# wondmgezahu/RAMP

Measured on AMD Instinct MI355X. Metric: sampled trajectories/sec (H=48, T=25), higher is better.
Workload: dtype f32-emulated (2 x fp16 planes per operand, fp32 accumulate)

## Files before the change

ramp_amd/csrc/tkc.hip:

```cpp
#include "args_conv.h"
#include "tokmma.h"

#include <algorithm>

namespace ramp {

namespace {

constexpr int tc_xrows(int NG) { return NG == 4 ? 64 + 2 + 2 : 48 + 2 * 6 + 2; }
constexpr int tc_scr(int NG) { return NG == 4 ? 2304 : 2048; }

__device__ __forceinline__ float tc_mish(float x) {
  const float e = __builtin_amdgcn_exp2f(fminf(x, 20.f) * 1.44269504088896340736f);
  const float n = e * (e + 2.f);
  return x * (n * __builtin_amdgcn_rcpf(n + 2.f));
}
__device__ __forceinline__ float tc_mish_grad(float x) {
  const float e = __builtin_amdgcn_exp2f(fminf(x, 20.f) * 1.44269504088896340736f);
  const float n = e * (e + 2.f);
  const float w = __builtin_amdgcn_rcpf(n + 2.f);
  return n * w + x * (4.f * e * (e + 1.f) * w * w);
}

__device__ __forceinline__ f32x4 tc_mm32(const u32x4 a, const u32x4 b, const f32x4 c) {
  return __builtin_amdgcn_mfma_f32_16x16x32_f16(__builtin_bit_cast(half8, a), __builtin_bit_cast(half8, b), c, 0, 0, 0);
}
__device__ __forceinline__ void tc_wave_sync() {
  __builtin_amdgcn_fence(__ATOMIC_ACQ_REL, "wavefront");
  __builtin_amdgcn_wave_barrier();
}

}

__global__ void tkc_pack_kernel(const float* __restrict__ W, unsigned short* __restrict__ out, int N, int K, float scale) {
  const int total = 5 * (N / 16) * (K / 32) * 64;
  const int idx = blockIdx.x * 256 + threadIdx.x;
  if (idx >= total) return;
  const int lane = idx & 63, f = idx >> 6;
  const int j = f % (K / 32), nb = (f / (K / 32)) % (N / 16), tap = f / ((K / 32) * (N / 16));
  const float* src = W + ((long)tap * N + 16 * nb + (lane & 15)) * K + 32 * j + 8 * (lane >> 4);
  unsigned short* o = out + (long)f * 1024 + lane * 8;
#pragma unroll
  for (int e = 0; e < 8; ++e) {
    const float x = src[e] * scale;
    const _Float16 hi = (_Float16)x, lo = (_Float16)(x - (float)hi);
    o[e] = __builtin_bit_cast(unsigned short, hi); o[512 + e] = __builtin_bit_cast(unsigned short, lo);
  }
}
int tkc_pack(const float* W, int N, int K, float scale, unsigned short* out, hipStream_t s) {
  RAMP_REQUIRE(W && out && N % 16 == 0 && K % 32 == 0 && N >= 16 && N <= 64 && K >= 32 && K <= 64, "tkc_pack: bad shape");
  const int total = 5 * (N / 16) * (K / 32) * 64;
  hipLaunchKernelGGL(tkc_pack_kernel, dim3((total + 255) / 256), dim3(256), 0, s, W, out, N, K, scale);
  RAMP_HIP_CHECK(hipGetLastError());
  return 0;
}
size_t tkc_packed_halves(int N, int K) { return (size_t)5 * (N / 16) * (K / 32) * 1024; }

template <int NG, int NB, int KS, int PRO, int EPI>
__global__ __launch_bounds__(256) __attribute__((amdgpu_waves_per_eu(1, 2)))
void tkc_kernel(TkcArgs a, int n_tiles) {
  constexpr int T = 16 * NG, K = 32 * KS, N = 16 * NB;
  constexpr int XROW = 4 * K + 16;
  constexpr int WBYTES = 5 * NB * KS * 2048;
  constexpr int TC_XROWS = tc_xrows(NG), TC_SCR = tc_scr(NG);
  static_assert(8 * T * 4 + 8 * (NG == 4 ? 1 : 6) * 4 <= TC_SCR, "GroupNorm scratch");
  extern __shared__ __attribute__((aligned(16))) char smem[];
  const int tid = threadIdx.x, lane = tid & 63;
  const int wave = __builtin_amdgcn_readfirstlane(tid >> 6);
  const int c = lane & 15, g = lane >> 4;
  const int n_my = (n_tiles - (int)blockIdx.x + (int)gridDim.x - 1) / (int)gridDim.x;

  const bool exact = a.amax_in == nullptr;
  float s_in = scale_of(a.amax_in);
  float os = a.wsi / s_in;
  float amax = 0.f;

  for (int i = tid; i < WBYTES / 16; i += 256) reinterpret_cast<u32x4*>(smem)[i] = reinterpret_cast<const u32x4*>(a.W)[i];
  char* xt = smem + WBYTES + wave * (TC_XROWS * XROW);
  for (int i = lane; i < TC_XROWS * XROW / 16; i += 64) reinterpret_cast<u32x4*>(xt)[i] = u32x4{0u, 0u, 0u, 0u};
  float* const wscr = reinterpret_cast<float*>(smem + WBYTES + 4 * (TC_XROWS * XROW) + wave * TC_SCR);
  __syncthreads();

  int xrow[NG], smp[NG];
#pragma unroll
  for (int t = 0; t < NG; ++t) { smp[t] = (16 * t + c) / a.L; xrow[t] = (16 * t + c) + 2 * smp[t] + 2; }
  const int n_smp = T / a.L;
  auto tok_sums = [&](float (&v)[4][NG], int nblk, int C) __attribute__((always_inline)) {
    const int gsz = C >> 3;
#pragma unroll
    for (int b = 0; b < 4; ++b) {
      if (b < nblk) {
#pragma unroll
        for (int t = 0; t < NG; ++t) {
          float q = v[b][t];
          if (gsz == 8) q += __shfl_xor(q, 16);
          const int grp = gsz == 4 ? 4 * b + g : 2 * b + (g >> 1);
          if (gsz == 4 || !(g & 1)) wscr[grp * T + 16 * t + c] = q;
        }
      }
    }
    tc_wave_sync();
    if (lane < 8 * n_smp) {
      const int grp = lane / n_smp, sm = lane - grp * n_smp;
      double q = 0.0;
      for (int u = 0; u < a.L; ++u) q += (double)wscr[grp * T + sm * a.L + u];
      wscr[8 * T + lane] = (float)(q / (double)(a.L * gsz));
    }
    tc_wave_sync();
#pragma unroll
    for (int b = 0; b < 4; ++b) {
      if (b < nblk) {
#pragma unroll
        for (int t = 0; t < NG; ++t) {
          const int grp = gsz == 4 ? 4 * b + g : 2 * b + (g >> 1);
          v[b][t] = wscr[8 * T + grp * n_smp + smp[t]];
        }
      }
    }
    tc_wave_sync();
  };
  const int m_last = a.M - 1;
  const char* xbase = reinterpret_cast<const char*>(a.X);

  f32x4 xr[K / 16][NG];
  f32x4 cr[PRO ? K / 16 : 1][PRO ? NG : 1];
  float gmu[PRO ? K / 16 : 1][PRO ? NG : 1], grs[PRO ? K / 16 : 1][PRO ? NG : 1];
  auto load_x = [&](int tile) __attribute__((always_inline)) {
    int tk0 = tile * (4 * T) + wave * T + c;
    asm volatile("" : "+v"(tk0));
#pragma unroll
    for (int t = 0; t < NG; ++t) {
      const unsigned tk = (unsigned)min(tk0 + 16 * t, m_last);
      const char* row = xbase + ((size_t)tk * (unsigned)(4 * a.ldx) + 16u * (unsigned)g);
#pragma unroll
      for (int fb = 0; fb < K / 16; ++fb) xr[fb][t] = *reinterpret_cast<const f32x4*>(row + 64 * fb);
      if constexpr (PRO) {
        const char* crow = reinterpret_cast<const char*>(a.gn_c) + ((size_t)tk * (unsigned)(4 * K) + 16u * (unsigned)g);
        const unsigned srow = tk / (unsigned)a.L;
#pragma unroll
        for (int fb = 0; fb < K / 16; ++fb) {
          cr[fb][t] = *reinterpret_cast<const f32x4*>(crow + 64 * fb);
          const int grp = K == 32 ? 4 * fb + g : 2 * fb + (g >> 1);
          gmu[fb][t] = a.gn_stats[((size_t)srow * 8 + grp) * 2]; grs[fb][t] = a.gn_stats[((size_t)srow * 8 + grp) * 2 + 1];
        }
      }
// ... 136 lines not shown
          var[nb][t] = q;
        }
      tok_sums(var, NB, N);
#pragma unroll
      for (int nb = 0; nb < NB; ++nb) {
        const f32x4 gam = *reinterpret_cast<const f32x4*>(a.gamma + 16 * nb + 4 * g), bet = *reinterpret_cast<const f32x4*>(a.beta + 16 * nb + 4 * g);
        f32x4 tb = (EPI == 1 && a.tbias) ? *reinterpret_cast<const f32x4*>(a.tbias + 16 * nb + 4 * g) : f32x4{0.f, 0.f, 0.f, 0.f};
#pragma unroll
        for (int t = 0; t < NG; ++t) {
          if constexpr (EPI == 2) tb = *reinterpret_cast<const f32x4*>(tline[t] + 16 * nb);
          const float rstd = 1.f / sqrtf(var[nb][t] + a.eps);
          const bool live = full || tok0 + 16 * t + c < a.M;
          if (live && (16 * t + c) - smp[t] * a.L == 0 && (N == 32 || !(g & 1))) {
            const int grp = N == 32 ? 4 * nb + g : 2 * nb + (g >> 1);
            float* st = a.stats + ((size_t)(trow[t] / (unsigned)a.L) * 8 + grp) * 2;
            st[0] = mean[nb][t]; st[1] = rstd;
          }
          f32x4 v;
#pragma unroll
          for (int j = 0; j < 4; ++j) v[j] = tc_mish((acc[nb][t][j] - mean[nb][t]) * rstd * gam[j] + bet[j]) + tb[j];
          if (a.resid) v += *reinterpret_cast<const f32x4*>(a.resid + (size_t)trow[t] * a.ldr + 16 * nb + 4 * g);
          if (live) *reinterpret_cast<f32x4*>(a.Y + (size_t)trow[t] * a.ldy + 16 * nb + 4 * g) = v;
        }
      }
    } else {
    {
      unsigned trow[NG];
#pragma unroll
      for (int t = 0; t < NG; ++t) trow[t] = (unsigned)min(tok0 + 16 * t + c, m_last);
      f32x4 bq[NB];
#pragma unroll
      for (int nb = 0; nb < NB; ++nb) bq[nb] = a.bias ? *reinterpret_cast<const f32x4*>(a.bias + 16 * nb + 4 * g) : f32x4{0.f, 0.f, 0.f, 0.f};
      if (full) {
        f32x4 rz[NB][NG];
#pragma unroll
        for (int nb = 0; nb < NB; ++nb)
#pragma unroll
          for (int t = 0; t < NG; ++t) rz[nb][t] = f32x4{0.f, 0.f, 0.f, 0.f};
        if (a.resid) {
#pragma unroll
          for (int nb = 0; nb < NB; ++nb)
#pragma unroll
            for (int t = 0; t < NG; ++t) rz[nb][t] = *reinterpret_cast<const f32x4*>(a.resid + (size_t)trow[t] * a.ldr + 16 * nb + 4 * g);
        }
        if (a.resid2) {
#pragma unroll
          for (int nb = 0; nb < NB; ++nb)
#pragma unroll
            for (int t = 0; t < NG; ++t) rz[nb][t] += *reinterpret_cast<const f32x4*>(a.resid2 + (size_t)trow[t] * a.ldr2 + 16 * nb + 4 * g);
        }
#pragma unroll
        for (int nb = 0; nb < NB; ++nb)
#pragma unroll
          for (int t = 0; t < NG; ++t) *reinterpret_cast<f32x4*>(a.Y + (size_t)trow[t] * a.ldy + 16 * nb + 4 * g) = acc[nb][t] * os + bq[nb] + rz[nb][t];
      } else {
#pragma unroll
        for (int nb = 0; nb < NB; ++nb)
#pragma unroll
          for (int t = 0; t < NG; ++t) {
            f32x4 v = acc[nb][t] * os + bq[nb];
            if (a.resid) v += *reinterpret_cast<const f32x4*>(a.resid + (size_t)trow[t] * a.ldr + 16 * nb + 4 * g);
            if (a.resid2) v += *reinterpret_cast<const f32x4*>(a.resid2 + (size_t)trow[t] * a.ldr2 + 16 * nb + 4 * g);
            if (tok0 + 16 * t + c < a.M) *reinterpret_cast<f32x4*>(a.Y + (size_t)trow[t] * a.ldy + 16 * nb + 4 * g) = v;
          }
      }
    }
  }

    }
  amax = fmaxf(amax, __shfl_xor(amax, 32)); amax = fmaxf(amax, __shfl_xor(amax, 16)); amax = fmaxf(amax, __shfl_xor(amax, 8));
  amax = fmaxf(amax, __shfl_xor(amax, 4)); amax = fmaxf(amax, __shfl_xor(amax, 2)); amax = fmaxf(amax, __shfl_xor(amax, 1));
  __syncthreads();
  record_amax_block_guarded<true>(a.amax_out, amax, reinterpret_cast<float*>(smem + WBYTES), exact ? nullptr : a.range_flag, s_in, a.site);
}

bool tkc_applicable(int M, int L, int N, int K, int* ng) {
  int n = 0;
  if (L >= 8 && 48 % L == 0) n = 3; else if (L >= 8 && 32 % L == 0) n = 2; else if (L == 64 && !(N == 64 && K == 64)) n = 4;
  if (ng) *ng = n;
  return n != 0 && M > 0 && M % L == 0 && (N == 32 || N == 64) && (K == 32 || K == 64);
}

namespace {
template <int NG, int NB, int KS> size_t tkc_lds() { return (size_t)5 * NB * KS * 2048 + 4 * (size_t)tc_xrows(NG) * (4 * 32 * KS + 16) + 4 * tc_scr(NG); }
template <int NG, int NB, int KS, int PRO, int EPI> int tkc_go(const TkcArgs& a, int n_tiles, hipStream_t s) {
  const size_t lds = tkc_lds<NG, NB, KS>();
  const int per_cu = lds * 2 <= 160 * 1024 ? 2 : 1;
  const int nb = std::min(n_tiles, per_cu * device_cu_count());
  hipLaunchKernelGGL((tkc_kernel<NG, NB, KS, PRO, EPI>), dim3(nb), dim3(256), lds, s, a, n_tiles);
  RAMP_HIP_CHECK(hipGetLastError());
  return 0;
}
}

int launch_tkc(const TkcArgs& a, hipStream_t s) {
  auto al16 = [](const void* p) { return (reinterpret_cast<uintptr_t>(p) & 15) == 0; };
  int ng = 0;
  RAMP_REQUIRE(tkc_applicable(a.M, a.L, a.N, a.K, &ng), "tkc: C_in, C_out in {32, 64}, tokens per sample >= 8 dividing 48 or 32 (or 64, not 64 x 64 channels), whole samples");
  RAMP_REQUIRE(a.X && a.W && a.Y && (a.dir == 1 || a.dir == -1), "tkc: bad operand");
  RAMP_REQUIRE(al16(a.X) && al16(a.W) && al16(a.Y) && al16(a.bias) && al16(a.resid) && al16(a.resid2) && a.ldx % 4 == 0 && a.ldy % 4 == 0 &&
               a.ldr % 4 == 0 && a.ldr2 % 4 == 0 && a.ldx >= a.K && a.ldy >= a.N, "tkc: operands must be 16-byte aligned");
  RAMP_REQUIRE((long)a.M * a.ldx * 4 < (1l << 32), "tkc: 32-bit row offsets");
  RAMP_REQUIRE(!ranges_overlap(a.Y, ((size_t)(a.M - 1) * a.ldy + a.N) * 4, a.X, ((size_t)(a.M - 1) * a.ldx + a.K) * 4), "tkc: the output must not overlap the operand");
  const int T = 16 * ng, n_tiles = (a.M + 4 * T - 1) / (4 * T);
  const int pro = a.gn_c ? 1 : 0, epi = a.Cst ? (a.t_rows ? 2 : 1) : 0;
  RAMP_REQUIRE(!a.t_rows || (a.Cst && a.tbias && a.tt_stride > 0 && a.tt_stride % 4 == 0), "tkc: a row -> timestep table needs the GroupNorm epilogue, the time table and its stride (a multiple of 4 floats)");
  RAMP_REQUIRE(!(pro && epi), "tkc: the GroupNorm backward operand and the GroupNorm epilogue do not occur together");
  if (pro) RAMP_REQUIRE(a.gn_stats && a.gn_gamma && a.gn_beta && al16(a.gn_c) && al16(a.gn_gamma) && al16(a.gn_beta) && a.ldx >= a.K, "tkc: GroupNorm-backward operand incomplete");
  if (epi) RAMP_REQUIRE(a.stats && a.gamma && a.beta && a.bias && !a.resid2 && al16(a.Cst) && al16(a.gamma) && al16(a.beta) && al16(a.tbias), "tkc: GroupNorm epilogue incomplete");
#define TC_SHAPE(NGV, PROV, EPIV) \
    if (a.N == 64 && a.K == 64) return tkc_go<NGV, 4, 2, PROV, EPIV>(a, n_tiles, s); \
    if (a.N == 64 && a.K == 32) return tkc_go<NGV, 4, 1, PROV, EPIV>(a, n_tiles, s); \
    if (a.N == 32 && a.K == 64) return tkc_go<NGV, 2, 2, PROV, EPIV>(a, n_tiles, s); \
    return tkc_go<NGV, 2, 1, PROV, EPIV>(a, n_tiles, s);
#define TC_CASE(NGV) \
  if (ng == NGV) { \
    if (pro) { TC_SHAPE(NGV, 1, 0) } \
    if (epi == 2) { TC_SHAPE(NGV, 0, 2) } \
    if (epi) { TC_SHAPE(NGV, 0, 1) } \
    TC_SHAPE(NGV, 0, 0) \
  }
  TC_CASE(3) TC_CASE(2)
#undef TC_SHAPE
#define TC_SHAPE(NGV, PROV, EPIV) \
    if (a.N == 64 && a.K == 32) return tkc_go<NGV, 4, 1, PROV, EPIV>(a, n_tiles, s); \
    if (a.N == 32 && a.K == 64) return tkc_go<NGV, 2, 2, PROV, EPIV>(a, n_tiles, s); \
    if (a.N == 32 && a.K == 32) return tkc_go<NGV, 2, 1, PROV, EPIV>(a, n_tiles, s);
  TC_CASE(4)
#undef TC_CASE
#undef TC_SHAPE
  RAMP_REQUIRE(false, "tkc: variant not built");
}

int init_tkc_attributes() {
#define TC_ATTR1(NGV, NBV, KSV, PROV, EPIV) RAMP_HIP_CHECK(hipFuncSetAttribute(reinterpret_cast<const void*>(&tkc_kernel<NGV, NBV, KSV, PROV, EPIV>), hipFuncAttributeMaxDynamicSharedMemorySize, (int)tkc_lds<NGV, NBV, KSV>()))
#define TC_ATTR(NGV, NBV, KSV) TC_ATTR1(NGV, NBV, KSV, 0, 0); TC_ATTR1(NGV, NBV, KSV, 1, 0); TC_ATTR1(NGV, NBV, KSV, 0, 1); TC_ATTR1(NGV, NBV, KSV, 0, 2)
  TC_ATTR(3, 4, 2); TC_ATTR(3, 4, 1); TC_ATTR(3, 2, 2); TC_ATTR(3, 2, 1);
  TC_ATTR(2, 4, 2); TC_ATTR(2, 4, 1); TC_ATTR(2, 2, 2); TC_ATTR(2, 2, 1);
  TC_ATTR(4, 4, 1); TC_ATTR(4, 2, 2); TC_ATTR(4, 2, 1);
#undef TC_ATTR
#undef TC_ATTR1
  return 0;
}

}
```

ramp_amd/csrc/tkw.hip:

```cpp
#include "args_conv.h"
#include "tokmma.h"

#include <algorithm>

namespace ramp {

namespace {

constexpr int TW_TB = 96;
constexpr int TW_NT = 3;
constexpr int TW_SCRATCH = 4096 + 4 * 1024;

__device__ __forceinline__ float tw_mish(float x) {
  const float e = __builtin_amdgcn_exp2f(fminf(x, 20.f) * 1.44269504088896340736f);
  const float n = e * (e + 2.f);
  return x * (n * __builtin_amdgcn_rcpf(n + 2.f));
}
__device__ __forceinline__ float tw_mish_grad(float x) {
  const float e = __builtin_amdgcn_exp2f(fminf(x, 20.f) * 1.44269504088896340736f);
  const float n = e * (e + 2.f);
  const float w = __builtin_amdgcn_rcpf(n + 2.f);
  return n * w + x * (4.f * e * (e + 1.f) * w * w);
}
__device__ __forceinline__ void tw_wave_sync() {
  __builtin_amdgcn_fence(__ATOMIC_ACQ_REL, "wavefront");
  __builtin_amdgcn_wave_barrier();
}

struct TwGeom { int KC, n_chunks, rows, xrow, n_pass; size_t lds; };
#define LR_GROUPS_OK(KC_, K_) (((KC_) / 4) / ((K_) / 32) <= 8)

}

template <int MB, int PRO, int EPI, bool RT>
__device__ __forceinline__ void tkw_body(const TkwArgs& a, int n_tiles, int kc32, int n_chunks, int n_rows, int n_pass, int mulL) {
  extern __shared__ __attribute__((aligned(16))) char smem[];
  const int tid = threadIdx.x, lane = tid & 63;
  const int wave = __builtin_amdgcn_readfirstlane(tid >> 6);
  const int tok = lane & 31, kh = lane >> 5;
  const int KC = kc32 << 5;
  const int XROW = 4 * KC + 16;
  const int KS = KC >> 4;
  char* const scr = smem + (size_t)n_rows * XROW;
  float* const wscr = reinterpret_cast<float*>(scr + wave * 1024);

  const float s_in = scale_of(a.amax_in);
  const float os = a.wsi / s_in;
  float amax = 0.f;
  auto divL = [&](int t) __attribute__((always_inline)) { return (t * mulL) >> 16; };
  auto trow = [&](int t) __attribute__((always_inline)) { return t + 2 * divL(t) + 2; };

  for (int i = tid; i < n_rows * XROW / 16; i += 256) reinterpret_cast<u32x4*>(smem)[i] = u32x4{0u, 0u, 0u, 0u};
  float* const prm = reinterpret_cast<float*>(scr + 4096);
  auto load_prm = [&](int c0) __attribute__((always_inline)) {
    for (int i = tid; i < min(a.N, 256); i += 256) {
      const int c = c0 + i;
      prm[i] = a.bias[c]; prm[256 + i] = a.gamma[c]; prm[512 + i] = a.beta[c]; prm[768 + i] = a.tbias ? a.tbias[c] : 0.f;
    }
  };
  if (EPI >= 1) load_prm(0);
  __syncthreads();

  int boff[TW_NT];
#pragma unroll
  for (int tg = 0; tg < TW_NT; ++tg) boff[tg] = trow(32 * tg + tok) * XROW + 16 * kh;
  const int LR = KC >> 2;
  const int RP = 64 / LR;
  const int sl = lane % LR, sr = lane / LR;
  const int m_last = a.M - 1;

#pragma unroll 1
  for (int tile = (int)blockIdx.x; tile < n_tiles; tile += (int)gridDim.x) {
    const int tok0 = tile * TW_TB;
#pragma unroll 1
    for (int pass = 0; pass < n_pass; ++pass) {
      f32x16 acc[MB][TW_NT];
#pragma unroll
      for (int mb = 0; mb < MB; ++mb)
#pragma unroll
        for (int tg = 0; tg < TW_NT; ++tg)
#pragma unroll
          for (int i = 0; i < 16; ++i) acc[mb][tg][i] = 0.f;
      const int nb0 = pass * 128 * MB + wave * 32 * MB;

#pragma unroll 1
      for (int kc = 0; kc < n_chunks; ++kc) {
        if (pass > 0 || kc > 0 || tile != (int)blockIdx.x) __syncthreads();
        if (EPI == 2 && kc == 0 && (pass > 0 || tile != (int)blockIdx.x)) load_prm(pass * 256);
        if (n_chunks > 1 || pass == 0) {
          const int ch = kc * KC + 4 * sl;
          if constexpr (PRO == 0) {
#pragma unroll 1
            for (int it0 = 0; it0 < 24; it0 += 8 * RP) {
              f32x4 v[8];
#pragma unroll
              for (int u = 0; u < 8; ++u) {
                const int t = 24 * wave + it0 + u * RP + sr;
                const int tk = min(tok0 + t, m_last);
                const float* src = ch < a.K1 ? a.X + (size_t)tk * a.ldx + ch : a.X2 + (size_t)tk * a.ldx2 + (ch - a.K1);
                v[u] = (it0 + u * RP < 24 && !(a.ablate & 2)) ? *reinterpret_cast<const f32x4*>(src) : f32x4{0.f, 0.f, 0.f, 0.f};
              }
#pragma unroll
              for (int u = 0; u < 8; ++u) {
                if (it0 + u * RP < 24) {
                  const int t = 24 * wave + it0 + u * RP + sr;
                  const f32x4 x = (tok0 + t < a.M) ? v[u] : f32x4{0.f, 0.f, 0.f, 0.f};
                  amax = amax4(x, amax);
                  unsigned h0, h1, l0, l1;
                  split4(x * s_in, h0, h1, l0, l1);
                  char* dst = smem + trow(t) * XROW + 8 * sl;
                  *reinterpret_cast<u32x2*>(dst) = u32x2{h0, h1};
                  *reinterpret_cast<u32x2*>(dst + 2 * KC) = u32x2{l0, l1};
                }
              }
            }
          } else {
            constexpr int NW = PRO > 0 ? PRO : 1;
            const int G4 = (a.K >> 5);
            const int grp = ch / (a.K >> 3), gl = sl / G4;
            const int n_gl = LR / G4;
            const f32x4 gam = *reinterpret_cast<const f32x4*>(a.gn_gamma + ch), bet = *reinterpret_cast<const f32x4*>(a.gn_beta + ch);
            const float inv_cnt = 1.f / (float)(a.L * (a.K >> 3));
            const int n_it = a.L / RP;
            const int spp = NW / n_it;
            const int n_smp = TW_TB / a.L;
            const int sm_lo = (wave * n_smp) >> 2, sm_hi = ((wave + 1) * n_smp) >> 2;
#pragma unroll 1
            for (int sm0 = sm_lo; sm0 < sm_hi; sm0 += spp) {
              const int t_lo = sm0 * a.L;
              f32x4 dv[NW], hv[NW];
              float mu[NW], rs[NW];
              int u_s = 0, u_i = 0;
#pragma unroll
              for (int u = 0; u < NW; ++u) {
                const int tk = min(tok0 + t_lo + u * RP + sr, m_last);
                dv[u] = *reinterpret_cast<const f32x4*>(a.X + (size_t)tk * a.ldx + ch);
                hv[u] = *reinterpret_cast<const f32x4*>(a.gn_c + (size_t)tk * a.K + ch);
                const int srow = min(tok0 / a.L + sm0 + u_s, m_last / a.L);
                mu[u] = a.gn_stats[((size_t)srow * 8 + grp) * 2]; rs[u] = a.gn_stats[((size_t)srow * 8 + grp) * 2 + 1];
                if (++u_i == n_it) { u_i = 0; ++u_s; }
              }
              float p1[NW], p2[NW];
#pragma unroll
              for (int u = 0; u < NW; ++u) {
                float s1 = 0.f, s2 = 0.f;
#pragma unroll
                for (int j = 0; j < 4; ++j) {
                  const float h = (hv[u][j] - mu[u]) * rs[u];
                  const float d = dv[u][j] * tw_mish_grad(h * gam[j] + bet[j]) * gam[j];
                  hv[u][j] = h; dv[u][j] = d;
                  s1 += d; s2 += d * h;
                }
                p1[u] = s1; p2[u] = s2;
              }
              for (int b = 1; b < G4; b <<= 1) {
#pragma unroll
                for (int u = 0; u < NW; ++u) { p1[u] += __shfl_xor(p1[u], b); p2[u] += __shfl_xor(p2[u], b); }
              }
              for (int b = LR; b < 64; b <<= 1) {
#pragma unroll
                for (int u = 0; u < NW; ++u) { p1[u] += __shfl_xor(p1[u], b); p2[u] += __shfl_xor(p2[u], b); }
              }
              if (sr == 0 && sl == gl * G4) {
#pragma unroll
                for (int u = 0; u < NW; ++u) { wscr[(gl * 8 + u) * 2] = p1[u]; wscr[(gl * 8 + u) * 2 + 1] = p2[u]; }
              }
              tw_wave_sync();
              if (lane < n_gl * spp) {
                const int g2 = lane / spp, s2i = lane - g2 * spp;
                float t1 = 0.f, t2 = 0.f;
                for (int i2 = 0; i2 < n_it; ++i2) { t1 += wscr[(g2 * 8 + s2i * n_it + i2) * 2]; t2 += wscr[(g2 * 8 + s2i * n_it + i2) * 2 + 1]; }
                wscr[(g2 * 8 + s2i * n_it) * 2] = t1 * inv_cnt; wscr[(g2 * 8 + s2i * n_it) * 2 + 1] = t2 * inv_cnt;
              }
              tw_wave_sync();
              u_s = 0; u_i = 0;
#pragma unroll
              for (int u = 0; u < NW; ++u) {
                const float m1 = wscr[(gl * 8 + u_s * n_it) * 2], m2 = wscr[(gl * 8 + u_s * n_it) * 2 + 1];
                if (++u_i == n_it) { u_i = 0; ++u_s; }
                const int t = t_lo + u * RP + sr;
                const bool live = tok0 + t < a.M;
                f32x4 x;
#pragma unroll
                for (int j = 0; j < 4; ++j) x[j] = live ? (dv[u][j] - m1 - hv[u][j] * m2) * rs[u] : 0.f;
                amax = amax4(x, amax);
                unsigned h0, h1, l0, l1;
                split4(x * s_in, h0, h1, l0, l1);
                char* dst = smem + trow(t) * XROW + 8 * sl;
                *reinterpret_cast<u32x2*>(dst) = u32x2{h0, h1};
                *reinterpret_cast<u32x2*>(dst + 2 * KC) = u32x2{l0, l1};
              }
              tw_wave_sync();
            }
          }
        }
        __syncthreads();

        const int n_steps = 5 * KS;
        const int lks = 31 - __builtin_clz(KS);
        const size_t wtap = (size_t)(a.N >> 5) * (a.K >> 4) * 2048;
        const char* wbase = reinterpret_cast<const char*>(a.W) + ((size_t)(nb0 >> 5) * (a.K >> 4) + (size_t)kc * KS) * 2048 + lane * 16;
        const size_t wmb = (size_t)(a.K >> 4) * 2048;
        auto load_a = [&](u32x4 (&h)[MB], u32x4 (&l)[MB], int st) __attribute__((always_inline)) {
          const char* p = wbase + (size_t)(st >> lks) * wtap + (size_t)(st & (KS - 1)) * 2048;
#pragma unroll
          for (int mb = 0; mb < MB; ++mb) {
            h[mb] = *reinterpret_cast<const u32x4*>(p + mb * wmb);
            l[mb] = *reinterpret_cast<const u32x4*>(p + mb * wmb + 1024);
          }
        };
        auto load_b = [&](u32x4 (&h)[TW_NT], u32x4 (&l)[TW_NT], int st) __attribute__((always_inline)) {
          const int sh = a.dir * ((st >> lks) - 2) * XROW + 32 * (st & (KS - 1));
#pragma unroll
          for (int tg = 0; tg < TW_NT; ++tg) {
            const char* p = smem + boff[tg] + sh;
            h[tg] = *reinterpret_cast<const u32x4*>(p);
            l[tg] = *reinterpret_cast<const u32x4*>(p + 2 * KC);
          }
        };
        auto step = [&](const u32x4 (&uah)[MB], const u32x4 (&ual)[MB], const u32x4 (&ubh)[TW_NT], const u32x4 (&ubl)[TW_NT],
                        u32x4 (&nah)[MB], u32x4 (&nal)[MB], u32x4 (&nbh)[TW_NT], u32x4 (&nbl)[TW_NT], int nxt) __attribute__((always_inline)) {
          const int sc = min(nxt, n_steps - 1);
          const char* pa = wbase + (size_t)(sc >> lks) * wtap + (size_t)(sc & (KS - 1)) * 2048;
          const int shn = a.dir * ((sc >> lks) - 2) * XROW + 32 * (sc & (KS - 1));
          auto issue = [&](int q) __attribute__((always_inline)) {
            if (q < 2 * MB) {
              const u32x4 v = *reinterpret_cast<const u32x4*>(pa + (q >> 1) * wmb + (q & 1) * 1024);
              if (q & 1) nal[q >> 1] = v; else nah[q >> 1] = v;
            } else if (q < 2 * MB + 2 * TW_NT) {
              const int r = q - 2 * MB;
              const u32x4 v = *reinterpret_cast<const u32x4*>(smem + boff[r >> 1] + shn + (r & 1) * 2 * KC);
              if (r & 1) nbl[r >> 1] = v; else nbh[r >> 1] = v;
            }
          };
          int q = 0;
#pragma unroll
          for (int mb = 0; mb < MB; ++mb)
#pragma unroll
            for (int tg = 0; tg < TW_NT; ++tg) {
              f32x16 v = acc[mb][tg];
              v = mfma16(uah[mb], ubl[tg], v);
              issue(q++);
              __builtin_amdgcn_sched_barrier(0);
              v = mfma16(ual[mb], ubh[tg], v);
              issue(q++);
              __builtin_amdgcn_sched_barrier(0);
              v = mfma16(uah[mb], ubh[tg], v);
              issue(q++);
              __builtin_amdgcn_sched_barrier(0);
              acc[mb][tg] = v;
            }
        };
        u32x4 a0h[MB], a0l[MB], a1h[MB], a1l[MB], b0h[TW_NT], b0l[TW_NT], b1h[TW_NT], b1l[TW_NT];
        load_a(a0h, a0l, 0); load_b(b0h, b0l, 0);
        __builtin_amdgcn_sched_barrier(0);
#pragma unroll 1
        for (int st = (a.ablate & 1) ? n_steps : 0; st < n_steps; st += 2) {
          step(a0h, a0l, b0h, b0l, a1h, a1l, b1h, b1l, st + 1);
          step(a1h, a1l, b1h, b1l, a0h, a0l, b0h, b0l, st + 2);
        }
      }

      if (EPI == 0) {
#pragma unroll
        for (int tg = 0; tg < TW_NT; ++tg) {
          const int t = tok0 + 32 * tg + tok;
          const int tk = min(t, m_last);
#pragma unroll
          for (int mb = 0; mb < MB; ++mb)
#pragma unroll
            for (int q = 0; q < 4; ++q) {
              const int n = nb0 + 32 * mb + 8 * q + 4 * kh;
              f32x4 v = quad(acc[mb][tg], q) * os;
              if (a.bias) v += *reinterpret_cast<const f32x4*>(a.bias + n);
              if (a.resid) v += *reinterpret_cast<const f32x4*>(a.resid + (size_t)tk * a.ldr + n);
              if (a.resid2) v += *reinterpret_cast<const f32x4*>(a.resid2 + (size_t)tk * a.ldr2 + n);
              float* dst = n < a.N1 ? a.Y + (size_t)tk * a.ldy + n : a.Y2 + (size_t)tk * a.ldy2 + (n - a.N1);
              if (t < a.M && !(a.ablate & 4)) *reinterpret_cast<f32x4*>(dst) = v;
            }
        }
      } else {
        constexpr int NGW = EPI == 2 ? 1 : 2;
        const int poff = EPI == 2 ? pass * 256 : 0;
        const int gsz = a.N >> 3;
        const int n_smp = TW_TB / a.L;
        const double inv_cnt = 1.0 / (double)(a.L * gsz);
#pragma unroll
        for (int mb = 0; mb < MB; ++mb)
#pragma unroll
          for (int q = 0; q < 4; ++q) {
            const f32x4 b4 = *reinterpret_cast<const f32x4*>(prm + nb0 - poff + 32 * mb + 8 * q + 4 * kh);
#pragma unroll
            for (int tg = 0; tg < TW_NT; ++tg)
#pragma unroll
              for (int j = 0; j < 4; ++j) acc[mb][tg][4 * q + j] = acc[mb][tg][4 * q + j] * os + b4[j];
          }
#pragma unroll
        for (int tg = 0; tg < TW_NT; ++tg) {
          const int t = tok0 + 32 * tg + tok;
          const int tk = min(t, m_last);
#pragma unroll
          for (int mb = 0; mb < MB; ++mb)
#pragma unroll
            for (int q = 0; q < 4; ++q)
              if (t < a.M && !(a.ablate & 4)) *reinterpret_cast<f32x4*>(a.Cst + (size_t)tk * a.N + nb0 + 32 * mb + 8 * q + 4 * kh) = quad(acc[mb][tg], q);
        }
        float mean_t[NGW][TW_NT], rstd_t[NGW][TW_NT];
        float my_mean = 0.f, my_var = 0.f;
#pragma unroll
        for (int rnd = 0; rnd < 2; ++rnd) {
#pragma unroll
          for (int gi = 0; gi < NGW; ++gi)
#pragma unroll
            for (int tg = 0; tg < TW_NT; ++tg) {
              constexpr int NS = EPI == 2 ? 16 * MB : (MB == 2 ? 16 : 8);
              float s = 0.f;
              if (rnd == 0 && EPI == 2) {
                double sd = 0.0;
#pragma unroll
                for (int i = 0; i < NS; ++i) sd += (double)acc[i >> 4][tg][i & 15];
                s = (float)sd;
              } else if (rnd == 0) {
                float p[NS];
#pragma unroll
                for (int i = 0; i < NS; ++i) p[i] = MB == 2 ? acc[gi][tg][i] : acc[0][tg][8 * gi + i];
                s = tree_sum(p);
              } else {
#pragma unroll
                for (int i = 0; i < NS; ++i) {
                  const float d = (EPI == 2 ? acc[i >> 4][tg][i & 15] : (MB == 2 ? acc[gi][tg][i] : acc[0][tg][8 * gi + i])) - mean_t[gi][tg];
                  s += d * d;
                }
              }
              s += __shfl_xor(s, 32);
              if (kh == 0) wscr[gi * TW_TB + 32 * tg + tok] = s;
            }
          tw_wave_sync();
          if (lane < NGW * n_smp) {
            const int gi = lane / n_smp, sm = lane - gi * n_smp;
            double sd = 0.0;
            for (int u = 0; u < a.L; ++u) sd += (double)wscr[gi * TW_TB + sm * a.L + u];
            const float s = (float)(sd * inv_cnt);
            wscr[192 + lane] = s;
            if (rnd == 0) my_mean = s; else my_var = s;
          }
          tw_wave_sync();
#pragma unroll
          for (int gi = 0; gi < NGW; ++gi)
#pragma unroll
            for (int tg = 0; tg < TW_NT; ++tg) {
              const float r = wscr[192 + gi * n_smp + divL(32 * tg + tok)];
              if (rnd == 0) mean_t[gi][tg] = r; else rstd_t[gi][tg] = 1.f / sqrtf(r + a.eps);
            }
          tw_wave_sync();
        }
        if (lane < NGW * n_smp) {
          const int gi = lane / n_smp, sm = lane - gi * n_smp;
          if (tok0 + sm * a.L < a.M) {
            const int g = EPI == 2 ? (nb0 >> 6) : (nb0 >> 5) * (MB == 2 ? 1 : 2) + gi;
            float* st = a.stats + ((size_t)(tok0 / a.L + sm) * 8 + g) * 2;
            st[0] = my_mean; st[1] = 1.f / sqrtf(my_var + a.eps);
          }
        }
#pragma unroll
        for (int tg = 0; tg < TW_NT; ++tg) {
          const int t = tok0 + 32 * tg + tok;
          const int tk = min(t, m_last);
          const float* tline = nullptr;
          if constexpr (RT) tline = a.tbias + (size_t)a.t_rows[min(tok0 / a.L + divL(32 * tg + tok), m_last / a.L)] * (size_t)a.tt_stride;
#pragma unroll
          for (int mb = 0; mb < MB; ++mb)
#pragma unroll
            for (int q = 0; q < 4; ++q) {
              const int n = nb0 + 32 * mb + 8 * q + 4 * kh;
              const int gi = EPI == 2 ? 0 : MB == 2 ? mb : (q >> 1);
              const f32x4 gam = *reinterpret_cast<const f32x4*>(prm + 256 + n - poff), bet = *reinterpret_cast<const f32x4*>(prm + 512 + n - poff);
              f32x4 v;
#pragma unroll
              for (int j = 0; j < 4; ++j) v[j] = tw_mish((acc[mb][tg][4 * q + j] - mean_t[gi][tg]) * rstd_t[gi][tg] * gam[j] + bet[j]);
              if constexpr (RT) v += *reinterpret_cast<const f32x4*>(tline + n);
              else v += *reinterpret_cast<const f32x4*>(prm + 768 + n - poff);
              if (a.resid) v += *reinterpret_cast<const f32x4*>(a.resid + (size_t)tk * a.ldr + n);
              if (t < a.M && !(a.ablate & 4)) *reinterpret_cast<f32x4*>(a.Y + (size_t)tk * a.ldy + n) = v;
            }
        }
      }
    }
  }

  amax = fmaxf(amax, __shfl_xor(amax, 32)); amax = fmaxf(amax, __shfl_xor(amax, 16)); amax = fmaxf(amax, __shfl_xor(amax, 8));
  amax = fmaxf(amax, __shfl_xor(amax, 4)); amax = fmaxf(amax, __shfl_xor(amax, 2)); amax = fmaxf(amax, __shfl_xor(amax, 1));
  record_amax_block_guarded<true>(a.amax_out, amax, reinterpret_cast<float*>(scr), a.range_flag, s_in, a.site);
}

template <int PRO, int EPI>
__global__ __launch_bounds__(256) __attribute__((amdgpu_waves_per_eu(2, 2)))
void tkw_kernel1(TkwArgs a, int n_tiles, int kc32, int n_chunks, int n_rows, int n_pass, int mulL) { tkw_body<1, PRO, EPI, false>(a, n_tiles, kc32, n_chunks, n_rows, n_pass, mulL); }
template <int PRO, int EPI>
__global__ __launch_bounds__(256) __attribute__((amdgpu_waves_per_eu(2, 2)))
void tkw_kernel2(TkwArgs a, int n_tiles, int kc32, int n_chunks, int n_rows, int n_pass, int mulL) { tkw_body<2, PRO, EPI, false>(a, n_tiles, kc32, n_chunks, n_rows, n_pass, mulL); }
template <int MB, int EPI>
__global__ __launch_bounds__(256) __attribute__((amdgpu_waves_per_eu(2, 2)))
void tkw_rows_kernel(TkwArgs a, int n_tiles, int kc32, int n_chunks, int n_rows, int n_pass, int mulL) { tkw_body<MB, 0, EPI, true>(a, n_tiles, kc32, n_chunks, n_rows, n_pass, mulL); }

namespace {

bool tw_geometry(int L, int N, int K, TwGeom* g) {
  if (L < 3 || TW_TB % L != 0) return false;
  if (!(N == 128 || N == 256 || N == 512 || N == 1024)) return false;
  if (K < 32 || K > 1024 || (K & (K - 1)) != 0) return false;
  const int rows = TW_TB + 2 * (TW_TB / L + 1);
  int KC = std::min(K, 128);
  while (KC > 32 && (size_t)rows * (4 * KC + 16) + TW_SCRATCH > 80 * 1024) KC >>= 1;
  if (KC < 32 || K % KC != 0) return false;
  g->KC = KC; g->n_chunks = K / KC; g->rows = rows; g->xrow = 4 * KC + 16;
  g->n_pass = N <= 256 ? 1 : N / 256;
  g->lds = (size_t)rows * g->xrow + TW_SCRATCH;
  return g->lds <= 80 * 1024;
}

int tw_pro_variant(int L, int N, int K) {
  TwGeom g;
  if (!tw_geometry(L, N, K, &g)) return 0;
  const int RP = 64 / (g.KC / 4);
  if (L % RP != 0 || (K / 8) % 4 != 0) return 0;
  const int n_it = L / RP, n_smp = TW_TB / L;
  for (int nw : {6, 8, 4, 3}) {
    if (nw % n_it != 0) continue;
    const int spp = nw / n_it;
    bool ok = true;
    for (int w = 0; w < 4; ++w) ok &= ((((w + 1) * n_smp) >> 2) - ((w * n_smp) >> 2)) % spp == 0;
    if (ok && (LR_GROUPS_OK(g.KC, K))) return nw;
  }
  return 0;
}

template <int MB, int PRO, int EPI, bool RT = false> int tkw_go(const TkwArgs& a, const TwGeom& g, hipStream_t s) {
  const int n_tiles = (a.M + TW_TB - 1) / TW_TB;
  const int per_cu = g.lds * 2 <= 160 * 1024 ? 2 : 1;
  const int nb = std::min(n_tiles, per_cu * device_cu_count());
  if constexpr (RT) hipLaunchKernelGGL((tkw_rows_kernel<MB, EPI ? EPI : 1>), dim3(nb), dim3(256), g.lds, s, a, n_tiles, g.KC >> 5, g.n_chunks, g.rows, g.n_pass, (65536 + a.L - 1) / a.L);
  else if (MB == 1) hipLaunchKernelGGL((tkw_kernel1<PRO, EPI>), dim3(nb), dim3(256), g.lds, s, a, n_tiles, g.KC >> 5, g.n_chunks, g.rows, g.n_pass, (65536 + a.L - 1) / a.L);
  else hipLaunchKernelGGL((tkw_kernel2<PRO, EPI>), dim3(nb), dim3(256), g.lds, s, a, n_tiles, g.KC >> 5, g.n_chunks, g.rows, g.n_pass, (65536 + a.L - 1) / a.L);
  RAMP_HIP_CHECK(hipGetLastError());
  return 0;
}

}

namespace { int tw_pro_variant(int L, int N, int K); }
bool tkw_applicable(int M, int L, int N, int K, int pro, int epi) {
  TwGeom g;
  if (!(M > 0 && M % L == 0 && tw_geometry(L, N, K, &g))) return false;
  if ((long)M * std::max(N, K) * 4 >= (1l << 32)) return false;
  if (pro) {
    if (tw_pro_variant(L, N, K) == 0) return false;
    if (g.n_chunks > 1 && (K / 8) > g.KC) return false;
  }
  if (epi && N > 512) return false;
  return true;
}

int launch_tkw(const TkwArgs& a, hipStream_t s) {
  auto al16 = [](const void* p) { return (reinterpret_cast<uintptr_t>(p) & 15) == 0; };
  const int pro = a.gn_c ? 1 : 0, epi = a.Cst ? 1 : 0;
  TwGeom g;
  RAMP_REQUIRE(tkw_applicable(a.M, a.L, a.N, a.K, pro, epi) && tw_geometry(a.L, a.N, a.K, &g),
               "tkw: C_out in {128, 256, 512, 1024} (<= 512 with the GroupNorm epilogue), C_in a power of two in [32, 1024], tokens per sample >= 3 dividing 96 (24 with the GroupNorm backward), whole samples");
  RAMP_REQUIRE(a.X && a.W && a.Y && (a.dir == 1 || a.dir == -1), "tkw: bad operand");
  RAMP_REQUIRE(a.K1 == a.K || (a.X2 && a.K1 > 0 && a.K1 < a.K && a.K1 % 4 == 0 && !pro), "tkw: bad operand split");
  RAMP_REQUIRE(a.N1 == a.N || (a.Y2 && a.N1 > 0 && a.N1 < a.N && a.N1 % 8 == 0 && !epi), "tkw: bad output split");
  RAMP_REQUIRE(al16(a.X) && al16(a.X2) && al16(a.W) && al16(a.Y) && al16(a.Y2) && al16(a.bias) && al16(a.resid) && al16(a.resid2) && al16(a.gn_c) &&
               al16(a.gn_gamma) && al16(a.gn_beta) && al16(a.Cst) && al16(a.gamma) && al16(a.beta) && al16(a.tbias) && a.ldx % 4 == 0 && a.ldx2 % 4 == 0 &&
               a.ldy % 4 == 0 && a.ldy2 % 4 == 0 && a.ldr % 4 == 0 && a.ldr2 % 4 == 0, "tkw: operands must be 16-byte aligned");
  if (pro) RAMP_REQUIRE(a.gn_stats && a.gn_gamma && a.gn_beta && a.ldx >= a.K, "tkw: GroupNorm-backward operand incomplete");
  if (epi) RAMP_REQUIRE(a.stats && a.gamma && a.beta && a.bias && !a.resid2 && a.ldy >= a.N, "tkw: GroupNorm epilogue incomplete");
  RAMP_REQUIRE(!a.t_rows || (epi && a.tbias && a.tt_stride > 0 && a.tt_stride % 4 == 0), "tkw: a row -> timestep table needs the GroupNorm epilogue, the time table and its stride (a multiple of 4 floats)");
  const size_t ybytes = ((size_t)(a.M - 1) * a.ldy + a.N1) * 4, xbytes = ((size_t)(a.M - 1) * a.ldx + a.K1) * 4;
  RAMP_REQUIRE(!ranges_overlap(a.Y, ybytes, a.X, xbytes), "tkw: the output must not overlap the operand");
  RAMP_REQUIRE(!epi || !ranges_overlap(a.Cst, (size_t)a.M * a.N * 4, a.X, xbytes), "tkw: the stash must not overlap the operand");
  const int mbv = a.N == 128 ? 1 : 2;
  const int prov = pro ? tw_pro_variant(a.L, a.N, a.K) : 0;
  const int epv = epi ? (a.N == 512 ? 2 : 1) : 0;
  if (a.t_rows) {
    if (mbv == 1) return tkw_go<1, 0, 1, true>(a, g, s);
    return epv == 2 ? tkw_go<2, 0, 2, true>(a, g, s) : tkw_go<2, 0, 1, true>(a, g, s);
  }
#define TW_CASE(MBV, PROV, EPIV) if (mbv == MBV && prov == PROV && epv == EPIV) return tkw_go<MBV, PROV, EPIV>(a, g, s);
  TW_CASE(1, 0, 0) TW_CASE(1, 0, 1) TW_CASE(1, 3, 0) TW_CASE(1, 4, 0) TW_CASE(1, 6, 0) TW_CASE(1, 8, 0)
  TW_CASE(2, 0, 0) TW_CASE(2, 0, 1) TW_CASE(2, 0, 2) TW_CASE(2, 3, 0) TW_CASE(2, 4, 0) TW_CASE(2, 6, 0) TW_CASE(2, 8, 0)
#undef TW_CASE
  RAMP_REQUIRE(false, "tkw: variant not built");
}

int init_tkw_attributes() {
#define TW_ATTR(KV, PROV, EPIV) RAMP_HIP_CHECK(hipFuncSetAttribute(reinterpret_cast<const void*>(&KV<PROV, EPIV>), hipFuncAttributeMaxDynamicSharedMemorySize, 160 * 1024))
  TW_ATTR(tkw_kernel1, 0, 0); TW_ATTR(tkw_kernel1, 0, 1); TW_ATTR(tkw_kernel1, 3, 0); TW_ATTR(tkw_kernel1, 4, 0); TW_ATTR(tkw_kernel1, 6, 0); TW_ATTR(tkw_kernel1, 8, 0);
  TW_ATTR(tkw_kernel2, 0, 0); TW_ATTR(tkw_kernel2, 0, 1); TW_ATTR(tkw_kernel2, 0, 2); TW_ATTR(tkw_kernel2, 3, 0); TW_ATTR(tkw_kernel2, 4, 0); TW_ATTR(tkw_kernel2, 6, 0); TW_ATTR(tkw_kernel2, 8, 0);
#undef TW_ATTR
#define TW_ATTR_RT(MBV, EPIV) RAMP_HIP_CHECK(hipFuncSetAttribute(reinterpret_cast<const void*>(&tkw_rows_kernel<MBV, EPIV>), hipFuncAttributeMaxDynamicSharedMemorySize, 160 * 1024))
  TW_ATTR_RT(1, 1); TW_ATTR_RT(2, 1); TW_ATTR_RT(2, 2);
#undef TW_ATTR_RT
  return 0;
}

}
```

Baseline: 4126.

## Swizzle tkw LDS token rows by rotation and specialize kernels for KC=128

Adds a per-row rotation swizzle to the LDS staging layout in the tkw kernel: writes and B-operand reads now go through tw_off, which rotates byte offsets within a row by an amount tied to the token's sample. This is meant to reduce LDS bank conflicts between lanes reading different token rows. It also adds compile-time KC=128 kernel instantiations so address arithmetic can fold into constants, with KC-generic fallback kernels for other geometries. The cost is extra integer ops per LDS access and twice as many instantiated kernels.

```diff
diff --git a/ramp_amd/csrc/lds_layout.h b/ramp_amd/csrc/lds_layout.h
--- /dev/null
+++ b/ramp_amd/csrc/lds_layout.h
@@ -0,0 +1,16 @@
+#pragma once
+
+namespace ramp {
+namespace {
+
+constexpr int tw_xrow(int KC) { return 4 * KC + 16; }
+constexpr int tw_row(int t, int s) { return t + 2 * s + 2; }
+constexpr int tw_rot_mask(int KC) { return (4 * KC < 256 ? 4 * KC : 256) - 1; }
+struct TwRow { int base, rot; };
+constexpr TwRow tw_row_of(int t, int s, int c, int KC) { return TwRow{tw_row(t, s) * tw_xrow(KC), c - 32 * s}; }
+constexpr int tw_off(TwRow r, int b, int m) { return r.base + (b & ~m) + ((r.rot + b) & m); }
+
+constexpr int tc_xrow(int K) { return 4 * K + 16; }
+
+}
+}
diff --git a/ramp_amd/csrc/tkc.hip b/ramp_amd/csrc/tkc.hip
--- a/ramp_amd/csrc/tkc.hip
+++ b/ramp_amd/csrc/tkc.hip
@@ -1,4 +1,5 @@
 #include "args_conv.h"
+#include "lds_layout.h"
 #include "tokmma.h"
 
 #include <algorithm>
@@ -60,7 +61,7 @@
 __global__ __launch_bounds__(256) __attribute__((amdgpu_waves_per_eu(1, 2)))
 void tkc_kernel(TkcArgs a, int n_tiles) {
   constexpr int T = 16 * NG, K = 32 * KS, N = 16 * NB;
-  constexpr int XROW = 4 * K + 16;
+  constexpr int XROW = tc_xrow(K);
   constexpr int WBYTES = 5 * NB * KS * 2048;
   constexpr int TC_XROWS = tc_xrows(NG), TC_SCR = tc_scr(NG);
   static_assert(8 * T * 4 + 8 * (NG == 4 ? 1 : 6) * 4 <= TC_SCR, "GroupNorm scratch");
@@ -363,7 +364,7 @@
 }
 
 namespace {
-template <int NG, int NB, int KS> size_t tkc_lds() { return (size_t)5 * NB * KS * 2048 + 4 * (size_t)tc_xrows(NG) * (4 * 32 * KS + 16) + 4 * tc_scr(NG); }
+template <int NG, int NB, int KS> size_t tkc_lds() { return (size_t)5 * NB * KS * 2048 + 4 * (size_t)tc_xrows(NG) * tc_xrow(32 * KS) + 4 * tc_scr(NG); }
 template <int NG, int NB, int KS, int PRO, int EPI> int tkc_go(const TkcArgs& a, int n_tiles, hipStream_t s) {
   const size_t lds = tkc_lds<NG, NB, KS>();
   const int per_cu = lds * 2 <= 160 * 1024 ? 2 : 1;
diff --git a/ramp_amd/csrc/tkw.hip b/ramp_amd/csrc/tkw.hip
--- a/ramp_amd/csrc/tkw.hip
+++ b/ramp_amd/csrc/tkw.hip
@@ -1,7 +1,9 @@
 #include "args_conv.h"
+#include "lds_layout.h"
 #include "tokmma.h"
 
 #include <algorithm>
+#include <type_traits>
 
 namespace ramp {
 
@@ -32,14 +34,15 @@
 
 }
 
-template <int MB, int PRO, int EPI, bool RT>
+template <int MB, int PRO, int EPI, bool RT, int KCT>
 __device__ __forceinline__ void tkw_body(const TkwArgs& a, int n_tiles, int kc32, int n_chunks, int n_rows, int n_pass, int mulL) {
   extern __shared__ __attribute__((aligned(16))) char smem[];
   const int tid = threadIdx.x, lane = tid & 63;
   const int wave = __builtin_amdgcn_readfirstlane(tid >> 6);
   const int tok = lane & 31, kh = lane >> 5;
-  const int KC = kc32 << 5;
-  const int XROW = 4 * KC + 16;
+  const int KC = KCT ? KCT : kc32 << 5;
+  const int XROW = tw_xrow(KC);
+  const int rmask = tw_rot_mask(KC);
   const int KS = KC >> 4;
   char* const scr = smem + (size_t)n_rows * XROW;
   float* const wscr = reinterpret_cast<float*>(scr + wave * 1024);
@@ -48,7 +51,7 @@
   const float os = a.wsi / s_in;
   float amax = 0.f;
   auto divL = [&](int t) __attribute__((always_inline)) { return (t * mulL) >> 16; };
-  auto trow = [&](int t) __attribute__((always_inline)) { return t + 2 * divL(t) + 2; };
+  auto trow = [&](int t, int c) __attribute__((always_inline)) { return tw_row_of(t, divL(t), c, KC); };
 
   for (int i = tid; i < n_rows * XROW / 16; i += 256) reinterpret_cast<u32x4*>(smem)[i] = u32x4{0u, 0u, 0u, 0u};
   float* const prm = reinterpret_cast<float*>(scr + 4096);
@@ -61,9 +64,6 @@
   if (EPI >= 1) load_prm(0);
   __syncthreads();
 
-  int boff[TW_NT];
-#pragma unroll
-  for (int tg = 0; tg < TW_NT; ++tg) boff[tg] = trow(32 * tg + tok) * XROW + 16 * kh;
   const int LR = KC >> 2;
   const int RP = 64 / LR;
   const int sl = lane % LR, sr = lane / LR;
@@ -108,9 +108,11 @@
                   amax = amax4(x, amax);
                   unsigned h0, h1, l0, l1;
                   split4(x * s_in, h0, h1, l0, l1);
-                  char* dst = smem + trow(t) * XROW + 8 * sl;
-                  *reinterpret_cast<u32x2*>(dst) = u32x2{h0, h1};
-                  *reinterpret_cast<u32x2*>(dst + 2 * KC) = u32x2{l0, l1};
+                  const TwRow r = trow(t, 0);
+                  int sb = 8 * sl;
+                  asm volatile("" : "+v"(sb));
+                  *reinterpret_cast<u32x2*>(smem + tw_off(r, sb, rmask)) = u32x2{h0, h1};
+                  *reinterpret_cast<u32x2*>(smem + tw_off(r, sb + 2 * KC, rmask)) = u32x2{l0, l1};
                 }
               }
             }
@@ -186,9 +188,11 @@
                 amax = amax4(x, amax);
                 unsigned h0, h1, l0, l1;
                 split4(x * s_in, h0, h1, l0, l1);
-                char* dst = smem + trow(t) * XROW + 8 * sl;
-                *reinterpret_cast<u32x2*>(dst) = u32x2{h0, h1};
-                *reinterpret_cast<u32x2*>(dst + 2 * KC) = u32x2{l0, l1};
+                const TwRow r = trow(t, 0);
+                int sb = 8 * sl;
+                asm volatile("" : "+v"(sb));
+                *reinterpret_cast<u32x2*>(smem + tw_off(r, sb, rmask)) = u32x2{h0, h1};
+                *reinterpret_cast<u32x2*>(smem + tw_off(r, sb + 2 * KC, rmask)) = u32x2{l0, l1};
               }
               tw_wave_sync();
             }
@@ -209,27 +213,35 @@
             l[mb] = *reinterpret_cast<const u32x4*>(p + mb * wmb + 1024);
           }
         };
+        TwRow brow[TW_NT];
+        {
+          int ln = lane;
+          asm volatile("" : "+v"(ln));
+#pragma unroll
+          for (int tg = 0; tg < TW_NT; ++tg) brow[tg] = trow(32 * tg + (ln & 31), 16 * (ln >> 5));
+        }
         auto load_b = [&](u32x4 (&h)[TW_NT], u32x4 (&l)[TW_NT], int st) __attribute__((always_inline)) {
-          const int sh = a.dir * ((st >> lks) - 2) * XROW + 32 * (st & (KS - 1));
+          const char* p = smem + a.dir * ((st >> lks) - 2) * XROW;
+          const int kb = 32 * (st & (KS - 1));
 #pragma unroll
           for (int tg = 0; tg < TW_NT; ++tg) {
-            const char* p = smem + boff[tg] + sh;
-            h[tg] = *reinterpret_cast<const u32x4*>(p);
-            l[tg] = *reinterpret_cast<const u32x4*>(p + 2 * KC);
+            h[tg] = *reinterpret_cast<const u32x4*>(p + tw_off(brow[tg], kb, rmask));
+            l[tg] = *reinterpret_cast<const u32x4*>(p + tw_off(brow[tg], kb + 2 * KC, rmask));
           }
         };
         auto step = [&](const u32x4 (&uah)[MB], const u32x4 (&ual)[MB], const u32x4 (&ubh)[TW_NT], const u32x4 (&ubl)[TW_NT],
                         u32x4 (&nah)[MB], u32x4 (&nal)[MB], u32x4 (&nbh)[TW_NT], u32x4 (&nbl)[TW_NT], int nxt) __attribute__((always_inline)) {
           const int sc = min(nxt, n_steps - 1);
           const char* pa = wbase + (size_t)(sc >> lks) * wtap + (size_t)(sc & (KS - 1)) * 2048;
-          const int shn = a.dir * ((sc >> lks) - 2) * XROW + 32 * (sc & (KS - 1));
+          const char* pb = smem + a.dir * ((sc >> lks) - 2) * XROW;
+          const int kbn = 32 * (sc & (KS - 1));
           auto issue = [&](int q) __attribute__((always_inline)) {
             if (q < 2 * MB) {
               const u32x4 v = *reinterpret_cast<const u32x4*>(pa + (q >> 1) * wmb + (q & 1) * 1024);
               if (q & 1) nal[q >> 1] = v; else nah[q >> 1] = v;
             } else if (q < 2 * MB + 2 * TW_NT) {
               const int r = q - 2 * MB;
-              const u32x4 v = *reinterpret_cast<const u32x4*>(smem + boff[r >> 1] + shn + (r & 1) * 2 * KC);
+              const u32x4 v = *reinterpret_cast<const u32x4*>(pb + tw_off(brow[r >> 1], kbn + (r & 1) * 2 * KC, rmask));
               if (r & 1) nbl[r >> 1] = v; else nbh[r >> 1] = v;
             }
           };
@@ -393,15 +405,18 @@
   record_amax_block_guarded<true>(a.amax_out, amax, reinterpret_cast<float*>(scr), a.range_flag, s_in, a.site);
 }
 
-template <int PRO, int EPI>
-__global__ __launch_bounds__(256) __attribute__((amdgpu_waves_per_eu(2, 2)))
-void tkw_kernel1(TkwArgs a, int n_tiles, int kc32, int n_chunks, int n_rows, int n_pass, int mulL) { tkw_body<1, PRO, EPI, false>(a, n_tiles, kc32, n_chunks, n_rows, n_pass, mulL); }
-template <int PRO, int EPI>
-__global__ __launch_bounds__(256) __attribute__((amdgpu_waves_per_eu(2, 2)))
-void tkw_kernel2(TkwArgs a, int n_tiles, int kc32, int n_chunks, int n_rows, int n_pass, int mulL) { tkw_body<2, PRO, EPI, false>(a, n_tiles, kc32, n_chunks, n_rows, n_pass, mulL); }
-template <int MB, int EPI>
-__global__ __launch_bounds__(256) __attribute__((amdgpu_waves_per_eu(2, 2)))
-void tkw_rows_kernel(TkwArgs a, int n_tiles, int kc32, int n_chunks, int n_rows, int n_pass, int mulL) { tkw_body<MB, 0, EPI, true>(a, n_tiles, kc32, n_chunks, n_rows, n_pass, mulL); }
+#define TW_KERNEL(NAME, TPARAMS, BODY_ARGS) \
+  template <TPARAMS> __global__ __launch_bounds__(256) __attribute__((amdgpu_waves_per_eu(2, 2))) \
+  void NAME(TkwArgs a, int n_tiles, int kc32, int n_chunks, int n_rows, int n_pass, int mulL) { tkw_body<BODY_ARGS>(a, n_tiles, kc32, n_chunks, n_rows, n_pass, mulL); }
+#define TW_COMMA ,
+TW_KERNEL(tkw_kernel1, int PRO TW_COMMA int EPI, 1 TW_COMMA PRO TW_COMMA EPI TW_COMMA false TW_COMMA 128)
+TW_KERNEL(tkw_kernel2, int PRO TW_COMMA int EPI, 2 TW_COMMA PRO TW_COMMA EPI TW_COMMA false TW_COMMA 128)
+TW_KERNEL(tkw_kc_kernel1, int PRO TW_COMMA int EPI, 1 TW_COMMA PRO TW_COMMA EPI TW_COMMA false TW_COMMA 0)
+TW_KERNEL(tkw_kc_kernel2, int PRO TW_COMMA int EPI, 2 TW_COMMA PRO TW_COMMA EPI TW_COMMA false TW_COMMA 0)
+TW_KERNEL(tkw_rows_kernel, int MB TW_COMMA int EPI, MB TW_COMMA 0 TW_COMMA EPI TW_COMMA true TW_COMMA 128)
+TW_KERNEL(tkw_kc_rows_kernel, int MB TW_COMMA int EPI, MB TW_COMMA 0 TW_COMMA EPI TW_COMMA true TW_COMMA 0)
+#undef TW_KERNEL
+#undef TW_COMMA
 
 namespace {
 
@@ -439,9 +454,17 @@
   const int n_tiles = (a.M + TW_TB - 1) / TW_TB;
   const int per_cu = g.lds * 2 <= 160 * 1024 ? 2 : 1;
   const int nb = std::min(n_tiles, per_cu * device_cu_count());
-  if constexpr (RT) hipLaunchKernelGGL((tkw_rows_kernel<MB, EPI ? EPI : 1>), dim3(nb), dim3(256), g.lds, s, a, n_tiles, g.KC >> 5, g.n_chunks, g.rows, g.n_pass, (65536 + a.L - 1) / a.L);
-  else if (MB == 1) hipLaunchKernelGGL((tkw_kernel1<PRO, EPI>), dim3(nb), dim3(256), g.lds, s, a, n_tiles, g.KC >> 5, g.n_chunks, g.rows, g.n_pass, (65536 + a.L - 1) / a.L);
-  else hipLaunchKernelGGL((tkw_kernel2<PRO, EPI>), dim3(nb), dim3(256), g.lds, s, a, n_tiles, g.KC >> 5, g.n_chunks, g.rows, g.n_pass, (65536 + a.L - 1) / a.L);
+  const dim3 grid(nb), block(256);
+  const int mulL = (65536 + a.L - 1) / a.L;
+  if (g.KC == 128 && !(MB == 2 && PRO == 8)) {
+    if constexpr (RT) hipLaunchKernelGGL((tkw_rows_kernel<MB, EPI ? EPI : 1>), grid, block, g.lds, s, a, n_tiles, g.KC >> 5, g.n_chunks, g.rows, g.n_pass, mulL);
+    else if constexpr (MB == 1) hipLaunchKernelGGL((tkw_kernel1<PRO, EPI>), grid, block, g.lds, s, a, n_tiles, g.KC >> 5, g.n_chunks, g.rows, g.n_pass, mulL);
+    else if constexpr (PRO != 8) hipLaunchKernelGGL((tkw_kernel2<PRO, EPI>), grid, block, g.lds, s, a, n_tiles, g.KC >> 5, g.n_chunks, g.rows, g.n_pass, mulL);
+  } else {
+    if constexpr (RT) hipLaunchKernelGGL((tkw_kc_rows_kernel<MB, EPI ? EPI : 1>), grid, block, g.lds, s, a, n_tiles, g.KC >> 5, g.n_chunks, g.rows, g.n_pass, mulL);
+    else if constexpr (MB == 1) hipLaunchKernelGGL((tkw_kc_kernel1<PRO, EPI>), grid, block, g.lds, s, a, n_tiles, g.KC >> 5, g.n_chunks, g.rows, g.n_pass, mulL);
+    else hipLaunchKernelGGL((tkw_kc_kernel2<PRO, EPI>), grid, block, g.lds, s, a, n_tiles, g.KC >> 5, g.n_chunks, g.rows, g.n_pass, mulL);
+  }
   RAMP_HIP_CHECK(hipGetLastError());
   return 0;
 }
@@ -495,12 +518,14 @@
 
 int init_tkw_attributes() {
 #define TW_ATTR(KV, PROV, EPIV) RAMP_HIP_CHECK(hipFuncSetAttribute(reinterpret_cast<const void*>(&KV<PROV, EPIV>), hipFuncAttributeMaxDynamicSharedMemorySize, 160 * 1024))
-  TW_ATTR(tkw_kernel1, 0, 0); TW_ATTR(tkw_kernel1, 0, 1); TW_ATTR(tkw_kernel1, 3, 0); TW_ATTR(tkw_kernel1, 4, 0); TW_ATTR(tkw_kernel1, 6, 0); TW_ATTR(tkw_kernel1, 8, 0);
-  TW_ATTR(tkw_kernel2, 0, 0); TW_ATTR(tkw_kernel2, 0, 1); TW_ATTR(tkw_kernel2, 0, 2); TW_ATTR(tkw_kernel2, 3, 0); TW_ATTR(tkw_kernel2, 4, 0); TW_ATTR(tkw_kernel2, 6, 0); TW_ATTR(tkw_kernel2, 8, 0);
+#define TW_ATTRS(K1, K2) \
+  TW_ATTR(K1, 0, 0); TW_ATTR(K1, 0, 1); TW_ATTR(K1, 3, 0); TW_ATTR(K1, 4, 0); TW_ATTR(K1, 6, 0); TW_ATTR(K1, 8, 0); \
+  TW_ATTR(K2, 0, 0); TW_ATTR(K2, 0, 1); TW_ATTR(K2, 0, 2); TW_ATTR(K2, 3, 0); TW_ATTR(K2, 4, 0); TW_ATTR(K2, 6, 0)
+  TW_ATTRS(tkw_kernel1, tkw_kernel2); TW_ATTRS(tkw_kc_kernel1, tkw_kc_kernel2); TW_ATTR(tkw_kc_kernel2, 8, 0);
+  TW_ATTR(tkw_rows_kernel, 1, 1); TW_ATTR(tkw_rows_kernel, 2, 1); TW_ATTR(tkw_rows_kernel, 2, 2);
+  TW_ATTR(tkw_kc_rows_kernel, 1, 1); TW_ATTR(tkw_kc_rows_kernel, 2, 1); TW_ATTR(tkw_kc_rows_kernel, 2, 2);
+#undef TW_ATTRS
 #undef TW_ATTR
-#define TW_ATTR_RT(MBV, EPIV) RAMP_HIP_CHECK(hipFuncSetAttribute(reinterpret_cast<const void*>(&tkw_rows_kernel<MBV, EPIV>), hipFuncAttributeMaxDynamicSharedMemorySize, 160 * 1024))
-  TW_ATTR_RT(1, 1); TW_ATTR_RT(2, 1); TW_ATTR_RT(2, 2);
-#undef TW_ATTR_RT
   return 0;
 }
 
```

After: 4127, median of 2. About the same (+0.0%).
